# spdes/chirpgp

Measured on AMD Instinct MI355X. Metric: filter+smoother trial-steps/s (batch x T / wall), higher is better.
Workload: dtype f64; 1 GPU; C2: discrete EKF+EKS (demos/ekfs_mle.py model); d=4, T=10000, batch_per_gpu=1000, global_batch=1000, parallelism=trials sharded x1

## Files before the change

chirpgp_amd/csrc/cgp_walk4.hpp:

```cpp
#pragma once
#include <atomic>
#include "cgp_coop8.hpp"

namespace cgp {

constexpr int kWalkRec = 37;
constexpr int kWalkG = 0, kWalkC = 16, kWalkc = 32;
constexpr int kWalkAhead = 2;
static_assert(kWalk4LdsBytes == sizeof(double) * 64 * kWalkRec, "walk4_smoother_ok (cgp_route.hpp) budgets the records of walk4_smoother_kernel");
constexpr int kWalkMapDoubles = 40;
struct Walk4Operands { double g, C, c; };

CGP_DEV double blk_bcast0(double x) {
    return dpp_banks_f64<kRowRor12, 0x8>(dpp_banks_f64<kRowRor8, 0x4>(dpp_banks_f64<kRowRor4, 0x2>(x, x), x), x);
}

template <class Elem, int MODE = kWalkWhole, bool SEL = false>
__global__ void __launch_bounds__(64) walk4_smoother_kernel(SmootherIO io, ModelArgs ma) {
    static_assert(Elem::D == 4, "d = 4 kernel");
    static_assert(!(SEL && MODE == kWalkCompose), "pass 1 of the time-split form writes nothing");
    __shared__ double recs[64 * kWalkRec];
    __shared__ double selbuf[SEL ? 128 : 1];
    __shared__ double ghrule[SEL ? 2 * kGhMaxOrder : 1];
    const int lane = threadIdx.x;
    const int r = lane >> 4, b = (lane >> 2) & 3, q = lane & 3;
    const int64_t trial = (MODE == kWalkWhole) ? (int64_t)blockIdx.x : (int64_t)(blockIdx.x / (unsigned)io.segs);
    const int seg = (MODE == kWalkWhole) ? 0 : (int)(blockIdx.x % (unsigned)io.segs);
    if (trial >= io.B) return;

    Elem elem;
    elem.setup(ma, trial);
    if constexpr (SEL) { sel_stage_rule(io.sel, ghrule, lane); wave_lds_fence(); }
    if constexpr (Elem::USES_SIGMA) elem.sg.stage(dyn_lds(), lane, 64, 4);
    const int64_t T = io.T;
    const double* __restrict__ mfs = io.mfs + trial * T * 4;
    const double* __restrict__ Pfs = io.Pfs + trial * T * 16;
    double* __restrict__ mss = io.mss + trial * T * 4;
    double* __restrict__ Pss = io.Pss + trial * T * 16;
    OobWindow wPs, wms;
    wPs.init((MODE == kWalkCompose || !io.Pss) ? nullptr : Pss, T * 128); wms.init((MODE == kWalkCompose || !io.mss) ? nullptr : mss, T * 32);
    const int64_t hi_first = (MODE == kWalkWhole) ? T - 2 : T - 2 - 64 * (int64_t)seg * io.tiles_per_seg;
    const int64_t hi_stop = (MODE == kWalkWhole) ? 0 : max((int64_t)0, hi_first - 64 * (int64_t)io.tiles_per_seg + 1);
    if (hi_first < 0 && MODE != kWalkWhole) return;
    const unsigned offP = (unsigned)b * 128u + (unsigned)(4 * r + q) * 8u;
    const unsigned offm = (q == 0) ? (unsigned)b * 32u + (unsigned)r * 8u : kOobOffset;
    const int oGa = kWalkG + q * 4 + r, oGb = kWalkG + r * 4 + q, oC = kWalkC + r * 4 + q, oc = kWalkc + r;

    double Ps = Pfs[(T - 1) * 16 + ((r >= q) ? r * 4 + q : q * 4 + r)];
    double ms = mfs[(T - 1) * 4 + r];
    double Acc = (r == q) ? 1.0 : 0.0;
    if constexpr (MODE == kWalkCompose) { Ps = 0.0; ms = 0.0; }
    if (MODE != kWalkCompose && seg == 0) {
        if (lane < 16 && (!SEL || io.Pss)) Pss[(T - 1) * 16 + lane] = Pfs[(T - 1) * 16 + lane];
        if (lane < 4 && (!SEL || io.mss)) mss[(T - 1) * 4 + lane] = mfs[(T - 1) * 4 + lane];
        if constexpr (SEL) { if (lane == 0) sel_write(io.sel, ghrule, trial * T + T - 1, mfs[(T - 1) * 4 + io.sel.comp], Pfs[(T - 1) * 16 + io.sel.comp * 5]); }
    }
    const bool sel_var_lane = SEL && r == io.sel.comp && q == io.sel.comp, sel_mean_lane = SEL && r == io.sel.comp && q == 0;
    if constexpr (MODE == kWalkApply) {
        const double* __restrict__ maps = io.ws + trial * io.segs * kWalkMapDoubles;
        for (int s2 = 0; s2 < seg; s2++) {
            const double* __restrict__ mp_ = maps + s2 * kWalkMapDoubles;
            const double gA = mp_[q * 4 + r], Cs = mp_[16 + r * 4 + q], cs = mp_[32 + r];
            const double Wc = mfma4x4(Ps, gA, 0.0);
            ms = mfma4x4(gA, ms, cs);
            Ps = mfma4x4(gA, Wc, Cs);
        }
    }

    auto request = [&](int64_t base, Vec<4>& mf, Sym<4>& Pf) {
        const int64_t t = base + lane;
        load_vec<4>(mfs + (t >= 0 ? t : 0) * 4, mf);
        load_sym<4>(Pfs + (t >= 0 ? t : 0) * 16, Pf);
    };
    auto write_record = [&](bool valid, const Mat<4>& G, const Vec<4>& c, const Sym<4>& C) {
        double* mine = recs + lane * kWalkRec;
        CGP_UNROLL for (int a = 0; a < 4; a++) {
            CGP_UNROLL for (int k = 0; k < 4; k++) {
                mine[kWalkG + a * 4 + k] = valid ? G.a[a][k] : 0.0;
                mine[kWalkC + a * 4 + k] = valid ? C(a, k) : 0.0;
            }
            mine[kWalkc + a] = valid ? c.v[a] : 0.0;
        }
    };
    auto scan = [&]() {
        CGP_UNROLL for (int i = 3; i >= 0; i--) {
            const double* p3 = recs + (16 * i + 4 * b + 3) * kWalkRec;
            double M = p3[oGb], C = p3[oC], c = p3[oc];
            CGP_UNROLL for (int j = 2; j >= 0; j--) {
                double* pj = recs + (16 * i + 4 * b + j) * kWalkRec;
                const double g = pj[oGa], Cj = pj[oC], cj = pj[oc];
                M = mfma4x4(g, M, 0.0);
                c = mfma4x4(g, c, cj);
                const double Tt = mfma4x4(C, g, 0.0);
                C = mfma4x4(Tt, g, Cj);
                pj[oGb] = M; pj[oC] = C; pj[oc] = c;
            }
        }
    };
    auto walk = [&](int64_t base) {
        auto fetch = [&](int Q, Walk4Operands& o) {
            const double* p = recs + ((4 * Q + (MODE == kWalkCompose ? 0 : b)) & 63) * kWalkRec;
            o.g = p[oGa]; o.C = p[oC]; o.c = p[oc];
        };
        Walk4Operands ring[kWalkAhead + 1];
        CGP_UNROLL for (int a = 0; a < kWalkAhead; a++) fetch(15 - a, ring[a]);
        CGP_UNROLL for (int Q = 15; Q >= 0; Q--) {
            fetch(Q - kWalkAhead, ring[(15 - Q + kWalkAhead) % (kWalkAhead + 1)]);
            const Walk4Operands& cur = ring[(15 - Q) % (kWalkAhead + 1)];
            if constexpr (MODE == kWalkCompose) {
                Acc = mfma4x4(cur.g, Acc, 0.0);
                ms = mfma4x4(cur.g, ms, cur.c);
                const double Tt = mfma4x4(Ps, cur.g, 0.0);
                Ps = mfma4x4(cur.g, Tt, cur.C);
            } else {
                const double W = mfma4x4(Ps, cur.g, 0.0);
                const double msn = mfma4x4(cur.g, ms, cur.c);
                const double Psn = mfma4x4(cur.g, W, cur.C);
                const unsigned step = (unsigned)(base + 4 * Q);
                wPs.store(Psn, offP + step * 128u);
                wms.store(msn, offm + step * 32u);
                if constexpr (SEL) {
                    if (sel_var_lane) selbuf[64 + 4 * Q + b] = Psn;
                    if (sel_mean_lane) selbuf[4 * Q + b] = msn;
                }
                Ps = blk_bcast0(Psn);
                ms = blk_bcast0(msn);
            }
        }
    };

    Vec<4> mf; Sym<4> Pf;
    if constexpr (Elem::HAS_SPEC) {
        {
            Mat<4> G; Vec<4> c; Sym<4> C;
            request(hi_first - 63, mf, Pf);
            const bool valid = hi_first - 63 + lane >= 0;
            if (valid) elem.map(mf, Pf, G, c, C);
            write_record(valid, G, c, C);
            wave_lds_fence();
            request(hi_first - 127, mf, Pf);
        }
        for (int64_t hi = hi_first; hi >= hi_stop; hi -= 64) {
            const int64_t base = hi - 63;
            Vec<4> mf2; Sym<4> Pf2;
            request(base - 128, mf2, Pf2);
            Mat<4> G; Vec<4> c; Sym<4> C; bool ok;
            elem.map_spec(mf, Pf, G, c, C, ok);
            scan();
            wave_lds_fence();
            walk(base);
            wave_lds_fence();
            if constexpr (SEL) { if (base + lane >= 0) sel_write(io.sel, ghrule, trial * T + base + lane, selbuf[lane], selbuf[64 + lane]); }
            if (__builtin_expect(__builtin_amdgcn_ballot_w64(!ok) != 0, 0)) elem.map(mf, Pf, G, c, C);
            write_record(base - 64 + lane >= 0, G, c, C);
            wave_lds_fence();
            mf = mf2; Pf = Pf2;
        }
    } else {
        request(hi_first - 63, mf, Pf);
        for (int64_t hi = hi_first; hi >= hi_stop; hi -= 64) {
            const int64_t base = hi - 63;
            {
                Mat<4> G; Vec<4> c; Sym<4> C;
                const bool valid = base + lane >= 0;
                if (valid) elem.map(mf, Pf, G, c, C);
                write_record(valid, G, c, C);
            }
            wave_lds_fence();
            request(base - 64, mf, Pf);
            scan();
            wave_lds_fence();
            walk(base);
            wave_lds_fence();
            if constexpr (SEL) { if (base + lane >= 0) sel_write(io.sel, ghrule, trial * T + base + lane, selbuf[lane], selbuf[64 + lane]); }
        }
    }
    if constexpr (MODE == kWalkCompose) {
        double* __restrict__ out = io.ws + (trial * io.segs + seg) * kWalkMapDoubles;
        if (b == 0) {
            out[r * 4 + q] = Acc;
            out[16 + r * 4 + q] = Ps;
            if (q == 0) out[32 + r] = ms;
        }
    }
}

template <class Elem>
inline hipError_t launch_walk4_smoother(const SmootherIO& io, const SmootherLaunch& host, const ModelArgs& ma, hipStream_t stream) {
    if (io.B <= 0 || io.T <= 0) return hipSuccess;
    if (!walk4_smoother_ok(io.T, ma)) return hipErrorInvalidValue;
    return launch_walk_smoother<Elem, walk4_smoother_kernel<Elem, kWalkWhole, false>, walk4_smoother_kernel<Elem, kWalkWhole, true>,
                                walk4_smoother_kernel<Elem, kWalkCompose, false>, walk4_smoother_kernel<Elem, kWalkApply, false>,
                                walk4_smoother_kernel<Elem, kWalkApply, true>>(io, host, ma, stream, kWalkMapDoubles);
}

}
```

Measured before the change: 3.927 billion trial-steps/s.

## Defer walk stores one step, split first tile, shorten block broadcast

In the smoother's backward walk, each step's stores of Ps and ms are delayed by one iteration, so global writes issue after the next broadcast and stay off the serial MFMA dependency chain. Full tiles are peeled from the final partial tile so they can use scalar-offset stores (store_s) with Q-constant immediates, and the partial tile keeps the per-step address computation. The block broadcast drops from three DPP ops to two by merging the last two masks. Map is now called unconditionally, with validity applied only on the record write. This risks extra register pressure and larger code from duplicated lambda instantiations.

```diff
diff --git a/chirpgp_amd/csrc/cgp_walk4.hpp b/chirpgp_amd/csrc/cgp_walk4.hpp
--- a/chirpgp_amd/csrc/cgp_walk4.hpp
+++ b/chirpgp_amd/csrc/cgp_walk4.hpp
@@ -12,7 +12,8 @@
 struct Walk4Operands { double g, C, c; };
 
 CGP_DEV double blk_bcast0(double x) {
-    return dpp_banks_f64<kRowRor12, 0x8>(dpp_banks_f64<kRowRor8, 0x4>(dpp_banks_f64<kRowRor4, 0x2>(x, x), x), x);
+    const double y = dpp_banks_f64<kRowRor4, 0x2>(x, x);
+    return dpp_banks_f64<kRowRor8, 0xC>(y, y);
 }
 
 template <class Elem, int MODE = kWalkWhole, bool SEL = false>
@@ -97,12 +98,30 @@
             }
         }
     };
-    auto walk = [&](int64_t base) {
+    auto walk = [&](int64_t base, auto first) {
+        constexpr bool FIRST = decltype(first)::value;
         auto fetch = [&](int Q, Walk4Operands& o) {
             const double* p = recs + ((4 * Q + (MODE == kWalkCompose ? 0 : b)) & 63) * kWalkRec;
             o.g = p[oGa]; o.C = p[oC]; o.c = p[oc];
         };
+        unsigned oP = offP, om = offm;
+        if constexpr (!FIRST) asm volatile("" : "+v"(oP), "+v"(om));
+        auto put = [&](int Q, double Psq, double msq) {
+            if constexpr (FIRST) {
+                const unsigned step = (unsigned)(base + 4 * Q);
+                wPs.store(Psq, oP + step * 128u);
+                wms.store(msq, om + step * 32u);
+            } else {
+                wPs.store_s(Psq, oP + (unsigned)Q * 512u, (unsigned)base * 128u);
+                wms.store_s(msq, om + (unsigned)Q * 128u, (unsigned)base * 32u);
+            }
+            if constexpr (SEL) {
+                if (sel_var_lane) selbuf[64 + 4 * Q + b] = Psq;
+                if (sel_mean_lane) selbuf[4 * Q + b] = msq;
+            }
+        };
         Walk4Operands ring[kWalkAhead + 1];
+        double Psq = 0.0, msq = 0.0;
         CGP_UNROLL for (int a = 0; a < kWalkAhead; a++) fetch(15 - a, ring[a]);
         CGP_UNROLL for (int Q = 15; Q >= 0; Q--) {
             fetch(Q - kWalkAhead, ring[(15 - Q + kWalkAhead) % (kWalkAhead + 1)]);
@@ -116,31 +135,35 @@
                 const double W = mfma4x4(Ps, cur.g, 0.0);
                 const double msn = mfma4x4(cur.g, ms, cur.c);
                 const double Psn = mfma4x4(cur.g, W, cur.C);
-                const unsigned step = (unsigned)(base + 4 * Q);
-                wPs.store(Psn, offP + step * 128u);
-                wms.store(msn, offm + step * 32u);
-                if constexpr (SEL) {
-                    if (sel_var_lane) selbuf[64 + 4 * Q + b] = Psn;
-                    if (sel_mean_lane) selbuf[4 * Q + b] = msn;
-                }
                 Ps = blk_bcast0(Psn);
                 ms = blk_bcast0(msn);
-            }
-        }
-    };
-
+                if (Q < 15) {
+                    asm("" : "+v"(Psq) : "v"(Ps));
+                    asm("" : "+v"(msq) : "v"(ms));
+                    put(Q + 1, Psq, msq);
+                }
+                Psq = Psn; msq = msn;
+            }
+        }
+        if constexpr (MODE != kWalkCompose) put(0, Psq, msq);
+    };
+
+    auto tiles = [&](auto body) {
+        int64_t hi = hi_first;
+        for (; hi >= hi_stop && hi >= 63; hi -= 64) body(hi, std::false_type{});
+        if (hi >= hi_stop) body(hi, std::true_type{});
+    };
     Vec<4> mf; Sym<4> Pf;
     if constexpr (Elem::HAS_SPEC) {
         {
             Mat<4> G; Vec<4> c; Sym<4> C;
             request(hi_first - 63, mf, Pf);
-            const bool valid = hi_first - 63 + lane >= 0;
-            if (valid) elem.map(mf, Pf, G, c, C);
-            write_record(valid, G, c, C);
+            elem.map(mf, Pf, G, c, C);
+            write_record(hi_first - 63 + lane >= 0, G, c, C);
             wave_lds_fence();
             request(hi_first - 127, mf, Pf);
         }
-        for (int64_t hi = hi_first; hi >= hi_stop; hi -= 64) {
+        tiles([&](int64_t hi, auto first) {
             const int64_t base = hi - 63;
             Vec<4> mf2; Sym<4> Pf2;
             request(base - 128, mf2, Pf2);
@@ -148,32 +171,31 @@
             elem.map_spec(mf, Pf, G, c, C, ok);
             scan();
             wave_lds_fence();
-            walk(base);
+            walk(base, first);
             wave_lds_fence();
             if constexpr (SEL) { if (base + lane >= 0) sel_write(io.sel, ghrule, trial * T + base + lane, selbuf[lane], selbuf[64 + lane]); }
             if (__builtin_expect(__builtin_amdgcn_ballot_w64(!ok) != 0, 0)) elem.map(mf, Pf, G, c, C);
             write_record(base - 64 + lane >= 0, G, c, C);
             wave_lds_fence();
             mf = mf2; Pf = Pf2;
-        }
+        });
     } else {
         request(hi_first - 63, mf, Pf);
-        for (int64_t hi = hi_first; hi >= hi_stop; hi -= 64) {
+        tiles([&](int64_t hi, auto first) {
             const int64_t base = hi - 63;
             {
                 Mat<4> G; Vec<4> c; Sym<4> C;
-                const bool valid = base + lane >= 0;
-                if (valid) elem.map(mf, Pf, G, c, C);
-                write_record(valid, G, c, C);
+                elem.map(mf, Pf, G, c, C);
+                write_record(base + lane >= 0, G, c, C);
             }
             wave_lds_fence();
             request(base - 64, mf, Pf);
             scan();
             wave_lds_fence();
-            walk(base);
+            walk(base, first);
             wave_lds_fence();
             if constexpr (SEL) { if (base + lane >= 0) sel_write(io.sel, ghrule, trial * T + base + lane, selbuf[lane], selbuf[64 + lane]); }
-        }
+        });
     }
     if constexpr (MODE == kWalkCompose) {
         double* __restrict__ out = io.ws + (trial * io.segs + seg) * kWalkMapDoubles;
```

Result: no change. 3.921 billion trial-steps/s, median of 2 (-0.1%).
